# lingfeiwang/normalisr

Hardware: AMD Instinct MI355X
Metric: association tests/sec (gene x gene coex) (higher is better)
Workload: dtype i8 digits x i8 -> i32 exact, 46-bit fixed point, f64 combine (f64 residuals, sums of sq...

## Files before the change

### include/normalisr_hip.h

```cpp
#ifndef NORMALISR_HIP_H
#define NORMALISR_HIP_H

#include <stdint.h>

#ifdef __cplusplus
extern "C" {
#endif

#define NRM_F32 0
#define NRM_F64 1

#define NRM_OK 0
#define NRM_E_ARG -1
#define NRM_E_DEVICE -2
#define NRM_E_NUMERIC -3
#define NRM_E_UNSUPPORTED -4

#define NRM_ROW_TILE 128
#define NRM_K_TILE 16

#define NRM_PCOEF 20

int nrm_version(void);
const char* nrm_last_error(void);
// ... 14 lines not shown
					const double* d_c, int64_t nc, int64_t ldc, const double* d_dci, int rank,
					double* d_out, int64_t ldo, int64_t rows_pad,
					double* d_ss, double* d_coef, void* stream);

#define NRM_FIX_STRIDE 8
int nrm_residualize_q(const void* d_x, int x_dtype, int64_t rows, int64_t n, int64_t ldx,
					  const double* d_c, int64_t nc, int64_t ldc, const double* d_dci, int rank,
					  double* d_out, int64_t ldo, int64_t rows_pad, double* d_ss, double* d_coef,
					  int nslices, void* d_q, int32_t* d_exp, int64_t plane_pitch_bytes, const double* d_cmax, double* d_fix, void* stream);
int nrm_binnet_debug_buffer(void* d_stamps);
int nrm_residualize_q_chunked(const void* d_x, int x_dtype, int64_t rows, int64_t n, int64_t ldx,
							  const double* d_c, int64_t nc, int64_t ldc, const double* d_dci, int rank,
							  int64_t rows_pad, double* d_ss, int nslices, void* d_q, int32_t* d_exp,
							  int64_t chunk_ksteps, const double* d_cmax, double* d_fix, void* stream);

int nrm_gram_f64(const double* d_a, const double* d_b, int64_t m_pad, int64_t n_pad, int64_t k_pad,
				 int64_t lda, int64_t ldb, double* d_dot, int64_t ldd, int symmetric,
				 int64_t m_rows, int64_t n_rows, void* d_work, void* stream);
int nrm_gram_f64_band(const double* d_a, const double* d_b, int64_t m_pad, int64_t n_pad, int64_t k_pad,
					  int64_t lda, int64_t ldb, double* d_dot, int64_t ldd, int symmetric,
					  int64_t m_rows, int64_t n_rows, int64_t row0, int64_t row1, void* d_work, void* stream);
int64_t nrm_gram_workspace_bytes(void);

int64_t nrm_quant_bytes(int64_t rows_pad, int64_t k_pad, int nslices);
int nrm_quantize_rows(const double* d_x, int64_t rows_pad, int64_t k_pad, int64_t ldx, int nslices, void* d_q, int32_t* d_exp,
					  double* d_fix , int64_t n_cells , void* stream);
int nrm_gram_i8_band(const void* d_qa, const int32_t* d_ea, int64_t plane_a_bytes, const void* d_qb, const int32_t* d_eb,
					 int64_t plane_b_bytes, int64_t m_pad, int64_t n_pad, int64_t k_pad, int nslices, double* d_dot, int64_t ldd,
					 int symmetric, int64_t m_rows, int64_t n_rows, int64_t row0, int64_t row1, void* d_work, void* stream);
int nrm_gram_i8_chunk(const void* d_qa, const int32_t* d_ea, int64_t plane_a_bytes, const void* d_qb, const int32_t* d_eb,
					  int64_t plane_b_bytes, int64_t m_pad, int64_t n_pad, int64_t k_pad, int nslices, double* d_dot, int64_t ldd,
					  int symmetric, int64_t m_rows, int64_t n_rows, int accumulate, int64_t b_block_rows, int64_t b_block_stride_bytes,
					  int b_first, int b_count, void* d_work, void* stream);

typedef struct nrm_pvalue_plan {
	double a;
	double alpha;
	double ln_front;
	double umax;
	double coef[NRM_PCOEF];
} nrm_pvalue_plan;
int nrm_pvalue_plan_init(nrm_pvalue_plan* plan, double dof);
int nrm_pvalue_plan_init_many(const double* dof, int64_t count, double* out, int64_t pitch);
int nrm_pvalue_plan_fill_many(const double* dof, int64_t count, double* out, int64_t pitch);

int nrm_pvalues_from_r2(const double* d_r2, int64_t count, double dof, double* d_p, void* stream);

int nrm_assoc_sweep(const double* d_dot, int64_t ldd, const double* d_ssx, const double* d_ssy,
					int64_t nx, int64_t ny, int64_t n_cells, double dof, int symmetric, int stat_kind,
					void* d_p, void* d_stat, void* d_r, void* d_t, int out_dtype, int64_t ldo,
					int32_t* d_flags, int fix_nslices, const double* d_fixx, const double* d_fixy, double guard_tol, void* stream);
int nrm_assoc_sweep_band(const double* d_dot, int64_t ldd, const double* d_ssx, const double* d_ssy,
						 int64_t nx, int64_t ny, int64_t n_cells, double dof, int symmetric, int stat_kind,
						 void* d_p, void* d_stat, void* d_r, void* d_t, int out_dtype, int64_t ldo,
						 int32_t* d_flags, int64_t row0, int64_t row1, int fix_nslices, const double* d_fixx, const double* d_fixy,
						 double guard_tol, void* stream);

int nrm_assoc_sweep_mirror(const double* d_dot, int64_t ldd, const double* d_ssx, const double* d_ssy, int64_t mx, int64_t my,
						   int64_t n_cells, double dof, void* d_p, void* d_stat, int out_dtype, int64_t ldo, int64_t r0, int64_t c0,
						   int32_t* d_flags, int fix_nslices, const double* d_fixx, const double* d_fixy, double guard_tol, void* stream);

int nrm_alpha(const void* d_stat, int stat_dtype, int64_t ldg, int stat_kind, const double* d_ssx, int64_t n_cells,
			  const double* d_bx, const double* d_by, int64_t nx, int64_t ny, int64_t nc, void* d_alpha, int out_dtype,
			  void* stream);

int64_t nrm_design_products_workspace_doubles(int64_t rows, int64_t n_cells);
// ... 297 lines not shown
```

### normalisr_amd/_lib.py

```python
import ctypes
import os
import sys

HERE = os.path.dirname(os.path.abspath(__file__))
LIB_PATH = os.path.join(HERE, 'libnormalisr_hip.so')

NRM_F32, NRM_F64 = 0, 1
NRM_TSV_I64, NRM_TSV_I32, NRM_TSV_U8 = 16, 17, 18
NRM_I64, NRM_I32, NRM_U8, NRM_I16 = 16, 17, 18, 19
NRM_S1_COMMON, NRM_S1_SKIP = -2, -1
DESIGN_NOTONE, DESIGN_NEG, DESIGN_GT1, DESIGN_HAS1, DESIGN_NAN = 1, 2, 4, 8, 16
DESIGN_CSR_BAD = 5
NRM_E_ARG, NRM_E_DEVICE, NRM_E_NUMERIC, NRM_E_UNSUPPORTED = -1, -2, -3, -4
ROW_TILE, K_TILE, PCOEF, FIX_STRIDE = 128, 16, 20, 8

_i64, _i32, _vp, _dbl = ctypes.c_int64, ctypes.c_int, ctypes.c_void_p, ctypes.c_double


class PvaluePlan(ctypes.Structure):
	_fields_ = [('a', _dbl), ('alpha', _dbl), ('ln_front', _dbl), ('umax', _dbl), ('coef', _dbl * PCOEF)]


_SIGNATURES = {
	'nrm_version': ([], _i32),
	'nrm_last_error': ([], ctypes.c_char_p),
	'nrm_device_count': ([ctypes.POINTER(_i32)], _i32),
	'nrm_set_device': ([_i32], _i32),
	'nrm_release_cache': ([], _i32),
	'nrm_last_guard': ([ctypes.POINTER(_i64), ctypes.POINTER(_dbl)], _i32),
	'nrm_host_pin': ([_vp, _i64, _i32], _i32),
	'nrm_host_unpin': ([_vp], _i32),
	'nrm_copy_to_host': ([_vp, _vp, _i64, _vp], _i32),
	'nrm_host_alloc': ([ctypes.POINTER(_vp), _i64], _i32),
	'nrm_host_free': ([_vp], _i32),
	'nrm_fill_zero': ([_vp, _i64, _vp], _i32),
	'nrm_fill_i32': ([_vp, _i32, _i64, _vp], _i32),
	'nrm_copy_rows': ([_vp, _i64, _vp, _i64, _i64, _i64, _vp], _i32),
	'nrm_residualize': ([_vp, _i32, _i64, _i64, _i64, _vp, _i64, _i64, _vp, _i32, _vp, _i64, _i64, _vp, _vp, _vp], _i32),
	'nrm_residualize_q': ([_vp, _i32, _i64, _i64, _i64, _vp, _i64, _i64, _vp, _i32, _vp, _i64, _i64, _vp, _vp, _i32, _vp, _vp, _i64, _vp, _vp, _vp], _i32),
	'nrm_binnet_debug_buffer': ([_vp], _i32),
	'nrm_residualize_q_chunked': ([_vp, _i32, _i64, _i64, _i64, _vp, _i64, _i64, _vp, _i32, _i64, _vp, _i32, _vp, _vp, _i64, _vp, _vp, _vp], _i32),
	'nrm_gram_f64': ([_vp, _vp, _i64, _i64, _i64, _i64, _i64, _vp, _i64, _i32, _i64, _i64, _vp, _vp], _i32),
	'nrm_gram_f64_band': ([_vp, _vp, _i64, _i64, _i64, _i64, _i64, _vp, _i64, _i32, _i64, _i64, _i64, _i64, _vp, _vp], _i32),
	'nrm_gram_workspace_bytes': ([], _i64),
	'nrm_quant_bytes': ([_i64, _i64, _i32], _i64),
	'nrm_quantize_rows': ([_vp, _i64, _i64, _i64, _i32, _vp, _vp, _vp, _i64, _vp], _i32),
	'nrm_gram_i8_band': ([_vp, _vp, _i64, _vp, _vp, _i64, _i64, _i64, _i64, _i32, _vp, _i64, _i32, _i64, _i64, _i64, _i64, _vp, _vp], _i32),
	'nrm_gram_i8_chunk': ([_vp, _vp, _i64, _vp, _vp, _i64, _i64, _i64, _i64, _i32, _vp, _i64, _i32, _i64, _i64, _i32, _i64, _i64, _i32, _i32, _vp, _vp], _i32),
	'nrm_pvalue_plan_init': ([ctypes.POINTER(PvaluePlan), _dbl], _i32),
	'nrm_pvalue_plan_init_many': ([_vp, _i64, _vp, _i64], _i32),
	'nrm_pvalue_plan_fill_many': ([_vp, _i64, _vp, _i64], _i32),
	'nrm_pvalues_from_r2': ([_vp, _i64, _dbl, _vp, _vp], _i32),
	'nrm_assoc_sweep': ([_vp, _i64, _vp, _vp, _i64, _i64, _i64, _dbl, _i32, _i32, _vp, _vp, _vp, _vp, _i32, _i64, _vp, _i32, _vp, _vp, _dbl, _vp], _i32),
	'nrm_assoc_sweep_band': ([_vp, _i64, _vp, _vp, _i64, _i64, _i64, _dbl, _i32, _i32, _vp, _vp, _vp, _vp, _i32, _i64, _vp, _i64, _i64, _i32, _vp, _vp, _dbl, _vp], _i32),
	'nrm_assoc_sweep_mirror': ([_vp, _i64, _vp, _vp, _i64, _i64, _i64, _dbl, _vp, _vp, _i32, _i64, _i64, _i64, _vp, _i32, _vp, _vp, _dbl, _vp], _i32),
	'nrm_host_mirror_rows': ([_vp, _i64, _i32, _i64, _i64, _i32], _i32),
	'nrm_copy_rect_to_host': ([_vp, _i64, _vp, _i64, _i64, _i64, _vp], _i32),
	'nrm_single4_sweep': ([_vp, _vp, _i64, _vp, _vp, _i64, _i64, _i64, _i64, _dbl, _i32, _vp, _vp, _vp, _i32, _i64, _vp, _vp, _vp], _i32),
	'nrm_gram_i8_fix_dot': ([_vp, _i64, _vp, _vp, _i64, _i64, _i32, _i64, _vp], _i32),
	'nrm_single4_sweep_guarded': ([_vp, _vp, _i64, _vp, _vp, _i64, _i64, _i64, _i64, _dbl, _i32, _vp, _vp, _vp, _i32, _i64, _vp, _vp,
								  _vp, _vp, _dbl, _dbl, _i32, _dbl, _vp, _vp], _i32),
	'nrm_spd_prepare': ([_vp, _i64, _i64, _i64, _vp, _vp, _vp, _vp], _i32),
	'nrm_spd_start': ([_vp, _i64, _i32, _vp, _vp, _vp], _i32),
	'nrm_spd_transpose_residual': ([_vp, _i64, _vp, _vp, _vp, _vp], _i32),
	'nrm_spd_update': ([_vp, _vp, _i64, _vp], _i32),
	'nrm_spd_finish': ([_vp, _i64, _i64, _vp, _vp, _vp, _vp], _i32),
	'nrm_single4_design_scalars': ([_vp, _i64, _i64, _vp, _vp, _vp, _vp], _i32),
	'nrm_design_products_workspace_doubles': ([_i64, _i64], _i64),
	'nrm_design_products': ([_vp, _i32, _i64, _i64, _i64, _vp, _i64, _i64, _vp, _vp, _i32, _vp], _i32),
	'nrm_residualize_wide': ([_vp, _i32, _i64, _i64, _i64, _vp, _i64, _i64, _vp, _vp, _i32, _vp, _i64, _vp, _vp, _vp, _i32, _vp], _i32),
	'nrm_gram_skinny': ([_vp, _i32, _i64, _i64, _i64, _vp, _i64, _i64, _vp, _vp, _i64, _i64, _dbl, _vp, _vp], _i32),
	'nrm_gram_skinny_workspace_bytes': ([], _i64),
	'nrm_de_small_sweep': ([_vp, _vp, _vp, _i64, _i32, _vp, _i64, _i64, _i64, _dbl, _i32, _vp, _vp, _vp, _vp, _i32, _i64, _vp, _vp, _vp, _i32, _vp], _i32),
	'nrm_single1_sweep': ([_vp, _i64, _vp, _i64, _vp, _i64, _i64, _i64, _i64, _i32, _vp, _vp, _vp, _vp, _i32, _i64, _vp, _vp], _i32),
	'nrm_de_sparse_chunk': ([], _i64),
	'nrm_de_sparse_max_covariates': ([], _i64),
	'nrm_de_sparse_fused_covariates': ([], _i64),
	'nrm_de_sparse_ct_doubles': ([_i64, _i64, _i64], _i64),
	'nrm_de_sparse': ([_vp, _i32, _i64, _i64, _i64, _vp, _i64, _vp, _vp, _vp, _vp, _vp, _vp, _i64, _vp, _vp, _i64, _vp, _i64, _i32, _vp, _vp, _vp, _vp, _i64, _i64, _dbl, _vp, _vp], _i32),
	'nrm_design_count': ([_vp, _i32, _i64, _i64, _i64, _vp, _i64, _vp, _vp], _i32),
	'nrm_design_plan': ([_vp, _i64, _i64, _i64, _vp, _vp, _vp, _vp, _vp, _vp, _vp, _vp, _vp], _i32),
# ... 207 lines not shown
```

### normalisr_amd/csrc/nrm_gram_i8.hip

```cpp
#include <type_traits>
#include "nrm_gram_sched.h"
#include "nrm_digits.h"
#include "nrm_fix.h"

#define QK 32
#define QCHUNK 512
#define QD 3
#ifndef QI_EDGE
#define QI_EDGE 0
#endif
#ifndef QI_EXP
#define QI_EXP 0
#endif

typedef int i4_t __attribute__((ext_vector_type(4)));
typedef int i16_t __attribute__((ext_vector_type(16)));

template <bool HAZARD>
__device__ __forceinline__ void q_dma16_s(const char* sbase, unsigned lane16, unsigned lds_dst) {
	if (HAZARD)
		asm volatile("s_nop 4\n\ts_mov_b32 m0, %2\n\ts_nop 0\n\tglobal_load_lds_dwordx4 %1, %0" ::"s"(sbase), "v"(lane16), "s"(lds_dst) : "m0");
	else
		asm volatile("s_mov_b32 m0, %2\n\ts_nop 0\n\tglobal_load_lds_dwordx4 %1, %0" ::"s"(sbase), "v"(lane16), "s"(lds_dst) : "m0");
}

template <int NS>
__global__ void __launch_bounds__(256) k_quantize_rows(const double* __restrict__ X, int64_t kx, int64_t ldx, char* __restrict__ Q,
													   int64_t plane_bytes, int64_t nks, int* __restrict__ exps, double* __restrict__ fix, double n_cells) {
	constexpr int B = 8 * NS - 2;
	const int lane = threadIdx.x & 63;
	const int64_t row = (int64_t)blockIdx.x * 4 + (threadIdx.x >> 6);
	const double* x = X + row * ldx;
	double mx = 0.0, ssq = 0.0;
	for (int64_t k = (int64_t)lane * 2; k < kx; k += 128) {
		const d2_t v = *reinterpret_cast<const d2_t*>(x + k);
		mx = fmax(mx, fmax(fabs(v[0]), fabs(v[1])));
		ssq = fma(v[0], v[0], fma(v[1], v[1], ssq));
	}
#pragma unroll
	for (int o = 32; o > 0; o >>= 1) mx = fmax(mx, __shfl_xor(mx, o, 64));
	int e = 0;
	if (mx > 0.0 && mx < INFINITY) (void)frexp(mx, &e);
	const int sh = e - B;
	if (lane == 0) exps[row] = sh;
	const int64_t ib = row >> 5;
	const int r = (int)(row & 31);
	char* qrow = Q + (ib * nks) * 1024 + (2 * r) * 16;
	const int flip = (r >> 3) & 1;
	int dsum[NS - 1];
	unsigned dsq[NS - 1];
	unsigned long long dsq64[NS - 1];
	unsigned steps = 0;
#pragma unroll
	for (int s = 0; s < NS - 1; s++) {
		dsum[s] = 0;
		dsq[s] = 0u;
// ... 20 lines not shown
			dsum[s] = __builtin_amdgcn_sdot4((int)w[s], 0x01010101, dsum[s], false);
			dsq[s] = (unsigned)__builtin_amdgcn_sdot4((int)w[s], (int)w[s], (int)dsq[s], false);
		}
		if ((++steps & 0x7fff) == 0) {
#pragma unroll
			for (int s = 0; s < NS - 1; s++) {
				dsq64[s] += dsq[s];
				dsq[s] = 0u;
			}
		}
	}
	if (fix) {
		double S[5] = {0, 0, 0, 0, 0}, Q2[5] = {0, 0, 0, 0, 0};
#pragma unroll
		for (int s = 0; s < NS - 1; s++) {
			S[s] = (double)wave_sum_i32(dsum[s]);
			unsigned long long q = dsq64[s] + dsq[s];
#pragma unroll
			for (int o = 32; o > 0; o >>= 1) q += __shfl_xor(q, o, 64);
			Q2[s] = (double)q;
		}
#pragma unroll
		for (int o = 32; o > 0; o >>= 1) ssq += __shfl_xor(ssq, o, 64);
		if (lane == 0) nrm_fix_record<NS>(fix + row * NRM_FIX_STRIDE, S, Q2, sh, ssq, n_cells);
	}
}

struct BBlocks {
	int rows;
	int first, count;
	int64_t stride;
};

template <int NS>
__device__ __forceinline__ void gram_piece_i8(const char* __restrict__ QA, const char* __restrict__ QB, int64_t plane_a, int64_t plane_b,
											  int64_t nks, const int* __restrict__ ea, const int* __restrict__ eb, double* __restrict__ C,
											  int64_t ldc, int ti, int tj, int k0, int k1, double* __restrict__ slab, int m_rows, int n_rows,
											  int symmetric, int accumulate, int edge_tj, BBlocks bb, const char* lds, unsigned lds0) {
	constexpr int STAGE = 8 * NS * 1024;
	const int tid = threadIdx.x, lane = tid & 63;
	const int wid = __builtin_amdgcn_readfirstlane(tid >> 6);
	const int wm = wid >> 2, wn = wid & 3;
	const char* qb_t = QB + ((int64_t)tj * 4 * nks) * 1024;
	const int* eb_t = eb + tj * GN;
	if (bb.rows) {
		const int blk = tj * GN / bb.rows, within = tj * GN - blk * bb.rows, wb = (bb.first + blk) % bb.count;
		qb_t = QB + wb * bb.stride + ((int64_t)(within / 32) * nks) * 1024;
		eb_t = eb + wb * bb.rows + within;
	}
	const bool host = symmetric && ti == tj && ti < edge_tj;
	const bool hw = host && wm == 1 && wn < 2;
	const char* src_w = wid < 4 ? QA + (((int64_t)ti * 4 + wid) * nks) * 1024
								: (host && wid == 4) ? QB + ((int64_t)edge_tj * 4 * nks) * 1024 : qb_t + ((int64_t)(wid - 4) * nks) * 1024;
	const unsigned src_hi = (unsigned)__builtin_amdgcn_readfirstlane((int)((uint64_t)src_w >> 32)),
				   src_lo = (unsigned)__builtin_amdgcn_readfirstlane((int)(uint64_t)src_w);
	const char* src0 = reinterpret_cast<const char*>((uint64_t)src_hi << 32 | (uint64_t)src_lo);
	const unsigned lane16 = lane * 16;
	const int64_t plane = wid < 4 ? plane_a : plane_b;
	const unsigned dst0 = lds0 + wid * NS * 1024;
	auto issue_one = [&](int buf, int ks, int s, auto hazard) {
		if (QI_EXP & 1) return;
		if (QI_EXP & 2) ks &= 3;
		q_dma16_s<decltype(hazard)::value>(src0 + s * plane + (int64_t)ks * 1024, lane16, dst0 + buf * STAGE + s * 1024);
	};
	auto issue = [&](int buf, int ks) {
#pragma unroll
		for (int s = 0; s < NS; s++) issue_one(buf, ks, s, std::true_type{});
	};
	i16_t acc[NS][2];
	auto clear = [&]() {
#pragma unroll
		for (int w = 0; w < NS; w++)
#pragma unroll
			for (int i = 0; i < 2; i++)
#pragma unroll
				for (int j = 0; j < 16; j++) acc[w][i][j] = 0;
	};
	const int r = lane & 31;
	const int pos = (2 * r + ((lane >> 5) ^ ((r >> 3) & 1))) * 16;
	const bool diag = symmetric && ti == tj;
	const bool edge = QI_EDGE && !diag && tj * GN + 32 >= n_rows;
	const int a_blk = edge ? (wid & 3) : hw ? wn * 2 : wm * 2, b_blk = edge ? 0 : wn;
	const int b_slot = hw ? 4 : (host && wid == 0) ? 0 : 4 + b_blk;
	const int aoff = a_blk * NS * 1024 + pos;
	const int boff = b_slot * NS * 1024 + pos;
	const int row_w = ti * GM + a_blk * 32, col_w = hw ? edge_tj * GN : tj * GN + b_blk * 32;
	bool want[2];
#pragma unroll
	for (int i = 0; i < 2; i++) want[i] = row_w + i * 32 < m_rows && col_w < n_rows && (!diag || col_w + 31 >= row_w + i * 32);
	if (edge) {
		want[0] = want[0] && wid < 4;
		want[1] = false;
	}
	double* cbase;
	int64_t pitch;
	if (slab) {
		cbase = slab + ((hw ? wm * 2 : a_blk) * 32) * GN + b_blk * 32;
		pitch = GN;
	} else {
		cbase = C + (int64_t)row_w * ldc + col_w;
		pitch = ldc;
	}
	cbase += (int64_t)(4 * (lane >> 5)) * pitch + (lane & 31);
	const int* ea_l = ea + row_w + 4 * (lane >> 5);
	const int eb_l = hw ? eb[edge_tj * GN + (lane & 31)] : eb_t[b_blk * 32 + (lane & 31)];
	auto flush = [&](bool first) {
#pragma unroll
		for (int i = 0; i < 2; i++) {
			if (!want[i]) continue;
#pragma unroll
			for (int q = 0; q < 16; q++) {
				const int rr = i * 32 + (q & 3) + 8 * (q >> 2);
				long long lo = 0, hi = 0;
#pragma unroll
				for (int w = 0; w < NS; w++) {
					if (w < 3)
						lo += (long long)acc[w][i][q] << (8 * w);
					else
						hi += (long long)acc[w][i][q] << (8 * (w - 3));
				}
				double v = fma((double)hi, 16777216.0, (double)lo);
				v = ldexp(v, ea_l[rr] + eb_l + 8 * (NS - 1));
				double* o = cbase + (int64_t)rr * pitch;
				*o = (first && !(accumulate && !slab)) ? v : *o + v;
			}
		}
	};
	clear();
	__syncthreads();
	if (k0 >= k1) return;
	issue(0, k0);
	issue(1, min(k0 + 1, k1 - 1));
	int in_chunk = 0;
	bool first = true;
	auto kloop = [&](auto mask) {
	constexpr int MASK = decltype(mask)::value;
	for (int ks = k0; ks < k1; ks++) {
		const int buf = (ks - k0) % QD;
		asm volatile("s_waitcnt vmcnt(%0)" ::"i"(NS) : "memory");
		if (!(QI_EXP & 4)) __syncthreads();
		const char* st = lds + buf * STAGE;
		const int nbuf = (ks - k0 + 2) % QD, nks = min(ks + 2, k1 - 1);
		i4_t fa[NS][2], fb[NS];
		auto read_row = [&](int s) {
#pragma unroll
			for (int i = 0; i < 2; i++)
				if (MASK >> i & 1) fa[s][i] = *reinterpret_cast<const i4_t*>(st + aoff + (i * NS + s) * 1024);
			fb[NS - 1 - s] = *reinterpret_cast<const i4_t*>(st + boff + (NS - 1 - s) * 1024);
		};
		auto mfma_row = [&](int s, int t0, int t1) {
#pragma unroll
			for (int t = t0; t < t1; t++)
#pragma unroll
				for (int i = 0; i < 2; i++)
					if (MASK >> i & 1)
						acc[s + t - (NS - 1)][i] = __builtin_amdgcn_mfma_i32_32x32x32_i8(fa[s][i], fb[t], acc[s + t - (NS - 1)][i], 0, 0, 0);
		};
		auto dma = [&](int j) {
			__builtin_amdgcn_sched_barrier(0);
			issue_one(nbuf, nks, j, std::false_type{});
			__builtin_amdgcn_sched_barrier(0);
		};
		if (MASK) {
			read_row(0);
			read_row(1);
#pragma unroll
			for (int s = 0; s < NS - 1; s++) {
				mfma_row(s, NS - 1 - s, NS);
				dma(s);
				if (s + 2 < NS) read_row(s + 2);
			}
			mfma_row(NS - 1, 0, NS / 2);
			dma(NS - 1);
			mfma_row(NS - 1, NS / 2, NS);
		} else {
#pragma unroll
			for (int s = 0; s < NS; s++) dma(s);
		}
		if (MASK && ++in_chunk == QCHUNK && ks + 1 < k1) {
			flush(first);
			first = false;
			clear();
			in_chunk = 0;
		}
	}
	};
	if (QI_EDGE && want[0] && !want[1])
		kloop(std::integral_constant<int, 1>{});
	else if (want[0] || want[1])
		kloop(std::integral_constant<int, 3>{});
	else
		kloop(std::integral_constant<int, 0>{});
	asm volatile("s_waitcnt vmcnt(0)" ::: "memory");
	flush(first);
}

template <int NS>
__global__ void __launch_bounds__(512) k_gram_i8(const char* __restrict__ QA, const char* __restrict__ QB, int64_t plane_a, int64_t plane_b,
												 int64_t nks, const int* __restrict__ ea, const int* __restrict__ eb, double* __restrict__ C,
												 int64_t ldc, int symmetric, GramSched s, BBlocks bb) {
	__shared__ __attribute__((aligned(1024))) char lds[QD * 8 * NS * 1024];
	typedef __attribute__((address_space(3))) char* lds_ptr_t;
	const unsigned lds0 = __builtin_amdgcn_readfirstlane((unsigned)(size_t)(lds_ptr_t)lds);
	gram_for_each_piece(s, [&](int t, int k0, int k1, double* slab) {
		int ti, tj;
		gram_sched_coords(s, t, symmetric, ti, tj);
		gram_piece_i8<NS>(QA, QB, plane_a, plane_b, nks, ea, eb, C, ldc, ti, tj, k0, k1, slab, s.m_rows, s.n_rows, symmetric, s.accumulate, s.fold,
						  bb, lds, lds0);
	});
}

static int g_num_cu_q = 0;

extern "C" int64_t nrm_quant_bytes(int64_t rows_pad, int64_t k_pad, int nslices) {
	if (rows_pad < 0 || k_pad < 0 || nslices < 1) return 0;
	const int64_t nks = (k_pad + QK - 1) / QK;
	return (rows_pad / 32) * nks * 1024 * nslices;
}

extern "C" int nrm_quantize_rows(const double* d_x, int64_t rows_pad, int64_t k_pad, int64_t ldx, int nslices, void* d_q, int32_t* d_exp,
								 double* d_fix, int64_t n_cells, void* stream) {
	NRM_REQUIRE(nslices == 5 || nslices == 6, "nrm_quantize_rows: 5 or 6 slices");
	NRM_REQUIRE(rows_pad >= 0 && rows_pad % 32 == 0 && k_pad > 0 && k_pad % 16 == 0 && ldx >= k_pad && ldx % 2 == 0,
				"nrm_quantize_rows: rows must be padded to 32 (%d for nrm_gram_i8), cells to 16", GM);
	if (rows_pad == 0) return NRM_OK;
	NRM_REQUIRE(d_x && d_q && d_exp && (uintptr_t)d_x % 16 == 0 && (uintptr_t)d_q % 16 == 0, "nrm_quantize_rows: null or misaligned pointer");
	NRM_REQUIRE(!d_fix || (n_cells > 0 && n_cells <= k_pad && k_pad < (1 << 22)), "nrm_quantize_rows: row records need 0 < n_cells <= k_pad < 2^22");
	const int64_t nks = (k_pad + QK - 1) / QK;
	const int64_t plane = (rows_pad / 32) * nks * 1024;
	dim3 grid((unsigned)(rows_pad / 4));
	if (nslices == 5)
		hipLaunchKernelGGL(k_quantize_rows<5>, grid, dim3(256), 0, (hipStream_t)stream, d_x, k_pad, ldx, (char*)d_q, plane, nks, d_exp, d_fix, (double)n_cells);
	else
		hipLaunchKernelGGL(k_quantize_rows<6>, grid, dim3(256), 0, (hipStream_t)stream, d_x, k_pad, ldx, (char*)d_q, plane, nks, d_exp, d_fix, (double)n_cells);
	return nrm_check_launch("k_quantize_rows");
}

static int gram_i8_impl(const void* d_qa, const int32_t* d_ea, int64_t plane_a_bytes, const void* d_qb, const int32_t* d_eb,
						int64_t plane_b_bytes, int64_t m_pad, int64_t n_pad, int64_t k_pad, int nslices, double* d_dot, int64_t ldd,
						int symmetric, int64_t m_rows, int64_t n_rows, int64_t row0, int64_t row1, int accumulate, BBlocks bb, bool may_fold, void* d_work, void* stream) {
	NRM_REQUIRE(nslices == 5 || nslices == 6, "nrm_gram_i8: 5 or 6 slices");
	NRM_REQUIRE(m_pad >= 0 && n_pad >= 0 && k_pad > 0 && m_pad % GM == 0 && n_pad % GN == 0, "nrm_gram_i8: sizes must be padded to %d", GM);
	NRM_REQUIRE(ldd >= n_pad && ldd % 2 == 0, "nrm_gram_i8: pitch too small");
	NRM_REQUIRE(!symmetric || m_pad == n_pad, "nrm_gram_i8: symmetric needs square output");
	NRM_REQUIRE(row0 >= 0 && row0 <= row1 && row1 <= m_pad && row0 % (GSB * GM) == 0 && (row1 % (GSB * GM) == 0 || row1 == m_pad),
				"nrm_gram_i8_band: rows [row0, row1) must be cut at multiples of %d", GSB * GM);
	if (m_pad == 0 || n_pad == 0 || row0 == row1) return NRM_OK;
	NRM_REQUIRE(d_qa && d_qb && d_ea && d_eb && d_dot && d_work, "nrm_gram_i8: null pointer");
	if (g_num_cu_q == 0) {
		int dev = 0;
		NRM_HIP(hipGetDevice(&dev));
		NRM_HIP(hipDeviceGetAttribute(&g_num_cu_q, hipDeviceAttributeMultiprocessorCount, dev));
		if (g_num_cu_q <= 0) g_num_cu_q = 256;
	}
	const int64_t nks = (k_pad + QK - 1) / QK;
	const int64_t plane_a = plane_a_bytes ? plane_a_bytes : (m_pad / 32) * nks * 1024,
				  plane_b = plane_b_bytes ? plane_b_bytes : ((bb.rows ? bb.rows : n_pad) / 32) * nks * 1024;
	NRM_REQUIRE(plane_a >= (m_pad / 32) * nks * 1024 && plane_b >= ((bb.rows ? bb.rows : n_pad) / 32) * nks * 1024,
				"nrm_gram_i8: plane pitch smaller than the operand");
	GramSched s;
	if (may_fold && symmetric && !accumulate && bb.rows == 0 && d_qa == d_qb && d_ea == d_eb && plane_a == plane_b && !nrm_debug_is("gram_fold", "0"))
		NRM_TRY(gram_plan_fold(s, m_pad, n_pad, nks, symmetric, m_rows, n_rows, row0, row1, g_num_cu_q, (double*)d_work));
	else
		NRM_TRY(gram_plan(s, m_pad, n_pad, nks, symmetric, m_rows, n_rows, row0, row1, g_num_cu_q, (double*)d_work));
	s.accumulate = accumulate ? 1 : 0;
	if (nslices == 5)
		hipLaunchKernelGGL(k_gram_i8<5>, dim3((unsigned)s.nwg), dim3(512), 0, (hipStream_t)stream, (const char*)d_qa, (const char*)d_qb, plane_a,
						   plane_b, nks, d_ea, d_eb, d_dot, ldd, symmetric, s, bb);
	else
		hipLaunchKernelGGL(k_gram_i8<6>, dim3((unsigned)s.nwg), dim3(512), 0, (hipStream_t)stream, (const char*)d_qa, (const char*)d_qb, plane_a,
						   plane_b, nks, d_ea, d_eb, d_dot, ldd, symmetric, s, bb);
	if (s.tiles_al + s.tiles_sk > 0)
		hipLaunchKernelGGL(k_gram_fixup<1>, dim3((unsigned)(s.tiles_al + s.tiles_sk), GM / GFIX_ROWS), dim3(256), 0, (hipStream_t)stream, d_dot, ldd, symmetric, s);
	return nrm_check_launch("k_gram_i8");
}

extern "C" int nrm_gram_i8_band(const void* d_qa, const int32_t* d_ea, int64_t plane_a_bytes, const void* d_qb, const int32_t* d_eb,
								int64_t plane_b_bytes, int64_t m_pad, int64_t n_pad, int64_t k_pad, int nslices, double* d_dot, int64_t ldd,
								int symmetric, int64_t m_rows, int64_t n_rows, int64_t row0, int64_t row1, void* d_work, void* stream) {
	return gram_i8_impl(d_qa, d_ea, plane_a_bytes, d_qb, d_eb, plane_b_bytes, m_pad, n_pad, k_pad, nslices, d_dot, ldd, symmetric, m_rows, n_rows, row0,
						row1, 0, BBlocks{0, 0, 1, 0}, true, d_work, stream);
}

extern "C" int nrm_gram_i8_chunk(const void* d_qa, const int32_t* d_ea, int64_t plane_a_bytes, const void* d_qb, const int32_t* d_eb,
								 int64_t plane_b_bytes, int64_t m_pad, int64_t n_pad, int64_t k_pad, int nslices, double* d_dot, int64_t ldd,
								 int symmetric, int64_t m_rows, int64_t n_rows, int accumulate, int64_t b_block_rows, int64_t b_block_stride_bytes,
								 int b_first, int b_count, void* d_work, void* stream) {
	BBlocks bb{0, 0, 1, 0};
	if (b_block_rows) {
		NRM_REQUIRE(!symmetric && b_block_rows > 0 && b_block_rows % GN == 0 && n_pad % b_block_rows == 0 && b_count > 0 && b_first >= 0 &&
						b_first < b_count && n_pad / b_block_rows <= b_count && b_block_stride_bytes % 16 == 0 && b_block_rows < (1 << 30),
					"nrm_gram_i8_chunk: bad block description of operand B");
		bb = BBlocks{(int)b_block_rows, b_first, b_count, b_block_stride_bytes};
	}
	return gram_i8_impl(d_qa, d_ea, plane_a_bytes, d_qb, d_eb, plane_b_bytes, m_pad, n_pad, k_pad, nslices, d_dot, ldd, symmetric, m_rows, n_rows, 0,
						m_pad, accumulate, bb, false, d_work, stream);
}
```

### normalisr_amd/csrc/nrm_host_logic.h

```cpp
#pragma once
#include <algorithm>
#include <cmath>
#include <cstdint>
#include <cstring>
#include <mutex>
#include <vector>
#include "../../include/normalisr_hip.h"

#if defined(__HIPCC__)
#define NRM_HD __host__ __device__
#else
#define NRM_HD
#endif

void nrm_set_error(const char* fmt, ...);
#ifndef NRM_REQUIRE
#define NRM_REQUIRE(cond, ...)      \
	do {                            \
		if (!(cond)) {              \
			nrm_set_error(__VA_ARGS__); \
			return NRM_E_ARG;       \
		}                           \
	} while (0)
#endif
// ... 41 lines not shown
					li = 0;
					int len = h;
					while (t >= len) {
						t -= len;
						li++;
						len--;
					}
					lj = li + t;
				}
				ti = bi * GSB + li;
				tj = bj * GSB + lj;
				return;
			}
			t -= cnt;
		}
	}
	ti = 0;
	tj = 0;
}

struct GramSched {
	int m_rows, n_rows;
	int ntm, ntn;
	int nkt;
	int tiles_dp;
	int tiles_al;
	int parts;
	int tiles_sk;
	int units_per_wg;
	int nwg;
	int tile0;
	int accumulate;
	int fold;
	double* work;
};

NRM_HD inline __attribute__((always_inline)) void gram_sched_coords(const GramSched& s, int t, int symmetric, int& ti, int& tj) {
	if (!s.fold) {
		gram_tile_coords(s.tile0 + t, symmetric, s.ntm, s.ntn, ti, tj);
		return;
	}
	const int lead = s.fold;
	if (t < lead * (lead + 1) / 2)
		gram_tile_coords(t, 1, lead, lead, ti, tj);
	else
		ti = tj = lead;
}
NRM_HD inline bool gram_is_host(const GramSched& s, int ti, int tj) { return ti == tj && ti < s.fold; }

template <typename F>
NRM_HD inline __attribute__((always_inline)) void gram_pieces_of(const GramSched& s, int block, F piece) {
	const int per_xcd = s.nwg >> 3;
	const int p = (block & 7) * per_xcd + (block >> 3);
	int t_dp = p;
	bool al_todo = p < s.tiles_al * s.parts;
	int64_t u = (int64_t)p * s.units_per_wg;
	const int64_t total = (int64_t)s.tiles_sk * s.nkt;
	int64_t uend = u + s.units_per_wg;
	if (uend > total) uend = total;
	int sk_piece = 0;
	for (;;) {
		int t, k0, k1;
		double* slab = nullptr;
		if (t_dp < s.tiles_dp) {
			t = t_dp;
			k0 = 0;
			k1 = s.nkt;
			t_dp += s.nwg;
		} else if (al_todo) {
			al_todo = false;
			const int ta = p / s.parts, part = p - ta * s.parts;
			t = s.tiles_dp + ta;
			k0 = (int)((int64_t)s.nkt * part / s.parts);
			k1 = (int)((int64_t)s.nkt * (part + 1) / s.parts);
			slab = s.work + (int64_t)p * (GM * GN);
		} else if (u < uend) {
			const int ts = (int)(u / s.nkt);
			k0 = (int)(u - (int64_t)ts * s.nkt);
			int64_t k1l = k0 + (uend - u);
			k1 = k1l > s.nkt ? s.nkt : (int)k1l;
			t = s.tiles_dp + s.tiles_al + ts;
			u += k1 - k0;
			if (!(k0 == 0 && k1 == s.nkt)) slab = s.work + ((int64_t)s.tiles_al * s.parts + 2 * p + sk_piece) * (GM * GN);
			sk_piece++;
		} else {
			break;
		}
		piece(t, k0, k1, slab);
	}
}

static inline int64_t nrm_host_gram_workspace_doubles(int nwg) { return (int64_t)3 * nwg * GM * GN; }

static inline int64_t gram_tiles_before(int64_t bi, int symmetric, int64_t ntm, int64_t ntn) {
	const int64_t nbn = (ntn + GSB - 1) / GSB;
	int64_t t = 0;
	for (int64_t b = 0; b < bi; b++) {
		const int64_t h = std::min<int64_t>(GSB, ntm - b * GSB);
		for (int64_t bj = symmetric ? b : 0; bj < nbn; bj++) {
			const int64_t w = std::min<int64_t>(GSB, ntn - bj * GSB);
			t += (symmetric && b == bj) ? h * (h + 1) / 2 : h * w;
		}
	}
	return t;
}

static inline void gram_split_phases(GramSched& s, int64_t tiles) {
	const int64_t waves = tiles / s.nwg, rem = tiles - waves * s.nwg;
	s.tiles_dp = (int)(waves * s.nwg);
	s.parts = 1;
	s.tiles_al = 0;
	for (int parts = 2; parts <= 8 && s.nkt >= 8 * parts; parts *= 2)
		if (rem >= s.nwg / parts) {
			s.parts = parts;
			s.tiles_al = s.nwg / parts;
			break;
		}
	const int64_t sk = rem - s.tiles_al;
	s.tiles_sk = (int)sk;
	s.units_per_wg = (int)((sk * s.nkt + s.nwg - 1) / s.nwg);
}

static inline int gram_plan(GramSched& s, int64_t m_pad, int64_t n_pad, int64_t nkt, int symmetric, int64_t m_rows, int64_t n_rows, int64_t row0,
							int64_t row1, int nwg, double* work) {
	const int64_t ntm = m_pad / GM, ntn = n_pad / GN;
	NRM_REQUIRE((symmetric ? ntn * (ntn + 1) / 2 : ntm * ntn) < (1LL << 30), "nrm_gram: problem too large for one launch");
	const int64_t tile0 = gram_tiles_before(row0 / (GSB * GM), symmetric, ntm, ntn);
	const int64_t tiles = gram_tiles_before((row1 + GSB * GM - 1) / (GSB * GM), symmetric, ntm, ntn) - tile0;
	NRM_REQUIRE(tiles < (1LL << 30) && nkt < (1LL << 30), "nrm_gram: problem too large for one launch");
	s.tile0 = (int)tile0;
	s.accumulate = 0;
	s.fold = 0;
	s.m_rows = (int)((m_rows > 0 && m_rows < m_pad) ? m_rows : m_pad);
	s.n_rows = (int)((n_rows > 0 && n_rows < n_pad) ? n_rows : n_pad);
	s.ntm = (int)ntm;
	s.ntn = (int)ntn;
	s.nkt = (int)nkt;
	s.nwg = nwg - nwg % 8;
	gram_split_phases(s, tiles);
	s.work = work;
	return NRM_OK;
}

static inline int gram_plan_fold(GramSched& s, int64_t m_pad, int64_t n_pad, int64_t nkt, int symmetric, int64_t m_rows, int64_t n_rows, int64_t row0,
								 int64_t row1, int nwg, double* work) {
	const int rc = gram_plan(s, m_pad, n_pad, nkt, symmetric, m_rows, n_rows, row0, row1, nwg, work);
	if (rc != NRM_OK) return rc;
	const int valid = s.n_rows - (s.ntn - 1) * GN;
	if (symmetric && row0 == 0 && row1 == m_pad && s.ntn >= 2 && s.ntm == s.ntn && s.m_rows == s.n_rows && valid >= 1 && valid <= 32) {
		s.fold = s.ntn - 1;
		gram_split_phases(s, (int64_t)(s.ntn - 1) * s.ntn / 2 + 1);
	}
	return NRM_OK;
}

static const double kNrmH[] = {1.0,
							-0.02083333333333333333333,
							0.000390625,
							-0.000007879670965608465608466,
							1.696766579172178130511e-7,
							-3.805064191721906565657e-9,
							8.748377596315407304061e-11,
							-2.044523359411973817584e-12,
							4.833351797967704408319e-14,
							-1.152434101767385923873e-15,
// ... 118 lines not shown
```

Baseline: 5.630 billion.

## Chain DMA prefetch across consecutive gram pieces and restructure flush

Replaces the per-piece callback loop with a cursor that looks ahead to the next piece. While the current piece's last k-steps run, it issues the next piece's first loads into the rotating LDS buffers, so the per-piece barrier and pipeline refill are skipped. The flush now combines the i8 digit planes with f64 FMAs and batches the loads of old output values. Row exponents are staged through a small added LDS region. Timestamp instrumentation compiled under QI_PHASES is also added. Chaining adds phase bookkeeping and a small LDS increase, and it can be switched off with a debug flag.

```diff
diff --git a/include/normalisr_hip.h b/include/normalisr_hip.h
--- a/include/normalisr_hip.h
+++ b/include/normalisr_hip.h
@@ -70,6 +70,7 @@
 					  int64_t plane_b_bytes, int64_t m_pad, int64_t n_pad, int64_t k_pad, int nslices, double* d_dot, int64_t ldd,
 					  int symmetric, int64_t m_rows, int64_t n_rows, int accumulate, int64_t b_block_rows, int64_t b_block_stride_bytes,
 					  int b_first, int b_count, void* d_work, void* stream);
+int nrm_k2_debug_buffer(void* d_stamps);
 
 typedef struct nrm_pvalue_plan {
 	double a;
diff --git a/normalisr_amd/_lib.py b/normalisr_amd/_lib.py
--- a/normalisr_amd/_lib.py
+++ b/normalisr_amd/_lib.py
@@ -47,6 +47,7 @@
 	'nrm_quantize_rows': ([_vp, _i64, _i64, _i64, _i32, _vp, _vp, _vp, _i64, _vp], _i32),
 	'nrm_gram_i8_band': ([_vp, _vp, _i64, _vp, _vp, _i64, _i64, _i64, _i64, _i32, _vp, _i64, _i32, _i64, _i64, _i64, _i64, _vp, _vp], _i32),
 	'nrm_gram_i8_chunk': ([_vp, _vp, _i64, _vp, _vp, _i64, _i64, _i64, _i64, _i32, _vp, _i64, _i32, _i64, _i64, _i32, _i64, _i64, _i32, _i32, _vp, _vp], _i32),
+	'nrm_k2_debug_buffer': ([_vp], _i32),
 	'nrm_pvalue_plan_init': ([ctypes.POINTER(PvaluePlan), _dbl], _i32),
 	'nrm_pvalue_plan_init_many': ([_vp, _i64, _vp, _i64], _i32),
 	'nrm_pvalue_plan_fill_many': ([_vp, _i64, _vp, _i64], _i32),
diff --git a/normalisr_amd/csrc/nrm_gram_i8.hip b/normalisr_amd/csrc/nrm_gram_i8.hip
--- a/normalisr_amd/csrc/nrm_gram_i8.hip
+++ b/normalisr_amd/csrc/nrm_gram_i8.hip
@@ -12,6 +12,10 @@
 #ifndef QI_EXP
 #define QI_EXP 0
 #endif
+#ifndef QI_PHASES
+#define QI_PHASES 0
+#endif
+#define QP_MAX 16
 
 typedef int i4_t __attribute__((ext_vector_type(4)));
 typedef int i16_t __attribute__((ext_vector_type(16)));
@@ -22,6 +26,18 @@
 		asm volatile("s_nop 4\n\ts_mov_b32 m0, %2\n\ts_nop 0\n\tglobal_load_lds_dwordx4 %1, %0" ::"s"(sbase), "v"(lane16), "s"(lds_dst) : "m0");
 	else
 		asm volatile("s_mov_b32 m0, %2\n\ts_nop 0\n\tglobal_load_lds_dwordx4 %1, %0" ::"s"(sbase), "v"(lane16), "s"(lds_dst) : "m0");
+}
+
+__device__ __forceinline__ long long q_stamp() {
+#if QI_PHASES
+	long long t;
+	__builtin_amdgcn_sched_barrier(0);
+	asm volatile("s_memrealtime %0\n\ts_waitcnt lgkmcnt(0)" : "=s"(t)::"memory");
+	__builtin_amdgcn_sched_barrier(0);
+	return t;
+#else
+	return 0;
+#endif
 }
 
 template <int NS>
@@ -108,40 +124,57 @@
 	int64_t stride;
 };
 
-template <int NS>
-__device__ __forceinline__ void gram_piece_i8(const char* __restrict__ QA, const char* __restrict__ QB, int64_t plane_a, int64_t plane_b,
-											  int64_t nks, const int* __restrict__ ea, const int* __restrict__ eb, double* __restrict__ C,
-											  int64_t ldc, int ti, int tj, int k0, int k1, double* __restrict__ slab, int m_rows, int n_rows,
-											  int symmetric, int accumulate, int edge_tj, BBlocks bb, const char* lds, unsigned lds0) {
-	constexpr int STAGE = 8 * NS * 1024;
-	const int tid = threadIdx.x, lane = tid & 63;
-	const int wid = __builtin_amdgcn_readfirstlane(tid >> 6);
-	const int wm = wid >> 2, wn = wid & 3;
+__device__ __forceinline__ const char* gram_wave_src(const char* __restrict__ QA, const char* __restrict__ QB, int64_t nks, int ti, int tj, int symmetric,
+													 int edge_tj, const BBlocks& bb, int wid) {
 	const char* qb_t = QB + ((int64_t)tj * 4 * nks) * 1024;
-	const int* eb_t = eb + tj * GN;
 	if (bb.rows) {
 		const int blk = tj * GN / bb.rows, within = tj * GN - blk * bb.rows, wb = (bb.first + blk) % bb.count;
 		qb_t = QB + wb * bb.stride + ((int64_t)(within / 32) * nks) * 1024;
-		eb_t = eb + wb * bb.rows + within;
 	}
 	const bool host = symmetric && ti == tj && ti < edge_tj;
-	const bool hw = host && wm == 1 && wn < 2;
 	const char* src_w = wid < 4 ? QA + (((int64_t)ti * 4 + wid) * nks) * 1024
 								: (host && wid == 4) ? QB + ((int64_t)edge_tj * 4 * nks) * 1024 : qb_t + ((int64_t)(wid - 4) * nks) * 1024;
 	const unsigned src_hi = (unsigned)__builtin_amdgcn_readfirstlane((int)((uint64_t)src_w >> 32)),
 				   src_lo = (unsigned)__builtin_amdgcn_readfirstlane((int)(uint64_t)src_w);
-	const char* src0 = reinterpret_cast<const char*>((uint64_t)src_hi << 32 | (uint64_t)src_lo);
+	return reinterpret_cast<const char*>((uint64_t)src_hi << 32 | (uint64_t)src_lo);
+}
+
+struct PieceLink {
+	const char* src;
+	const char* tail;
+	int tail_mask;
+	int phase;
+	bool chained_in;
+};
+
+template <int NS>
+__device__ __forceinline__ void gram_piece_i8(const int* __restrict__ ea, const int* __restrict__ eb, int64_t plane_a, int64_t plane_b, double* __restrict__ C,
+											  int64_t ldc, int ti, int tj, int k0, int k1, double* __restrict__ slab, int m_rows, int n_rows,
+											  int symmetric, int accumulate, int edge_tj, BBlocks bb, PieceLink link, char* lds, unsigned lds0, long long* stamps, int piece_idx) {
+	constexpr int STAGE = 8 * NS * 1024;
+	const long long t_entry = q_stamp();
+	long long t_first = 0;
+	const int tid = threadIdx.x, lane = tid & 63;
+	const int wid = __builtin_amdgcn_readfirstlane(tid >> 6);
+	const int wm = wid >> 2, wn = wid & 3;
+	const int* eb_t = eb + tj * GN;
+	if (bb.rows) {
+		const int blk = tj * GN / bb.rows, within = tj * GN - blk * bb.rows, wb = (bb.first + blk) % bb.count;
+		eb_t = eb + wb * bb.rows + within;
+	}
+	const bool host = symmetric && ti == tj && ti < edge_tj;
+	const bool hw = host && wm == 1 && wn < 2;
+	const char* src0 = link.src;
 	const unsigned lane16 = lane * 16;
 	const int64_t plane = wid < 4 ? plane_a : plane_b;
 	const unsigned dst0 = lds0 + wid * NS * 1024;
-	auto issue_one = [&](int buf, int ks, int s, auto hazard) {
+	auto issue_one = [&](int buf, const char* src, int s, auto hazard) {
 		if (QI_EXP & 1) return;
-		if (QI_EXP & 2) ks &= 3;
-		q_dma16_s<decltype(hazard)::value>(src0 + s * plane + (int64_t)ks * 1024, lane16, dst0 + buf * STAGE + s * 1024);
+		q_dma16_s<decltype(hazard)::value>(src + s * plane, lane16, dst0 + buf * STAGE + s * 1024);
 	};
 	auto issue = [&](int buf, int ks) {
 #pragma unroll
-		for (int s = 0; s < NS; s++) issue_one(buf, ks, s, std::true_type{});
+		for (int s = 0; s < NS; s++) issue_one(buf, src0 + (int64_t)((QI_EXP & 2) ? ks & 3 : ks) * 1024, s, std::true_type{});
 	};
 	i16_t acc[NS][2];
 	auto clear = [&]() {
@@ -178,45 +211,67 @@
 		pitch = ldc;
 	}
 	cbase += (int64_t)(4 * (lane >> 5)) * pitch + (lane & 31);
-	const int* ea_l = ea + row_w + 4 * (lane >> 5);
+	const int ea_w = ea[row_w + ((QI_EDGE && edge) ? (lane & 31) : lane)];
 	const int eb_l = hw ? eb[edge_tj * GN + (lane & 31)] : eb_t[b_blk * 32 + (lane & 31)];
+	int* const ex_w = reinterpret_cast<int*>(lds + QD * STAGE) + wid * 64;
 	auto flush = [&](bool first) {
-#pragma unroll
-		for (int i = 0; i < 2; i++) {
-			if (!want[i]) continue;
-#pragma unroll
-			for (int q = 0; q < 16; q++) {
-				const int rr = i * 32 + (q & 3) + 8 * (q >> 2);
-				long long lo = 0, hi = 0;
-#pragma unroll
-				for (int w = 0; w < NS; w++) {
-					if (w < 3)
-						lo += (long long)acc[w][i][q] << (8 * w);
-					else
-						hi += (long long)acc[w][i][q] << (8 * (w - 3));
-				}
-				double v = fma((double)hi, 16777216.0, (double)lo);
-				v = ldexp(v, ea_l[rr] + eb_l + 8 * (NS - 1));
-				double* o = cbase + (int64_t)rr * pitch;
-				*o = (first && !(accumulate && !slab)) ? v : *o + v;
+		ex_w[lane] = ea_w;
+		const int* ex_l = ex_w + 4 * (lane >> 5);
+		auto value = [&](int i, int q) {
+			double lo = (double)acc[2][i][q], hi = (double)acc[NS - 1][i][q];
+			lo = fma(lo, 256.0, (double)acc[1][i][q]);
+			lo = fma(lo, 256.0, (double)acc[0][i][q]);
+#pragma unroll
+			for (int w = NS - 2; w >= 3; w--) hi = fma(hi, 256.0, (double)acc[w][i][q]);
+			const int rr = i * 32 + (q & 3) + 8 * (q >> 2);
+			return ldexp(fma(hi, 16777216.0, lo), ex_l[rr] + eb_l + 8 * (NS - 1));
+		};
+		if (first && !(accumulate && !slab)) {
+#pragma unroll
+			for (int i = 0; i < 2; i++) {
+				if (!want[i]) continue;
+#pragma unroll
+				for (int q = 0; q < 16; q++) cbase[(int64_t)(i * 32 + (q & 3) + 8 * (q >> 2)) * pitch] = value(i, q);
+			}
+		} else {
+#pragma unroll
+			for (int i = 0; i < 2; i++) {
+				if (!want[i]) continue;
+				double old[16];
+#pragma unroll
+				for (int q = 0; q < 16; q++) old[q] = cbase[(int64_t)(i * 32 + (q & 3) + 8 * (q >> 2)) * pitch];
+#pragma unroll
+				for (int q = 0; q < 16; q++) cbase[(int64_t)(i * 32 + (q & 3) + 8 * (q >> 2)) * pitch] = old[q] + value(i, q);
 			}
 		}
 	};
 	clear();
-	__syncthreads();
-	if (k0 >= k1) return;
-	issue(0, k0);
-	issue(1, min(k0 + 1, k1 - 1));
+	if (!link.chained_in) {
+		__syncthreads();
+		issue(0, k0);
+		issue(1, min(k0 + 1, k1 - 1));
+	}
 	int in_chunk = 0;
 	bool first = true;
+	if (QI_PHASES) {
+		asm volatile("s_waitcnt vmcnt(%0)" ::"i"(NS) : "memory");
+		__builtin_amdgcn_s_barrier();
+		t_first = q_stamp();
+	}
 	auto kloop = [&](auto mask) {
 	constexpr int MASK = decltype(mask)::value;
-	for (int ks = k0; ks < k1; ks++) {
-		const int buf = (ks - k0) % QD;
+	int ks = k0;
+#pragma nounroll
+	for (int pass = 0; pass < 2; pass++) {
+	const int kend = pass ? k1 : max(k0, k1 - 2);
+	const char* nsrc = pass ? link.tail + (int64_t)((ks + 2 - k1) & link.tail_mask) * 1024 : src0 + (int64_t)(k0 + 2) * 1024;
+	const int nstep = pass ? (1024 & link.tail_mask) : 1024;
+	for (; ks < kend; ks++, nsrc += nstep) {
+		const int buf = (ks - k0 + link.phase) % QD;
 		asm volatile("s_waitcnt vmcnt(%0)" ::"i"(NS) : "memory");
 		if (!(QI_EXP & 4)) __syncthreads();
 		const char* st = lds + buf * STAGE;
-		const int nbuf = (ks - k0 + 2) % QD, nks = min(ks + 2, k1 - 1);
+		const int nbuf = (ks - k0 + 2 + link.phase) % QD;
 		i4_t fa[NS][2], fb[NS];
 		auto read_row = [&](int s) {
 #pragma unroll
@@ -234,7 +289,7 @@
 		};
 		auto dma = [&](int j) {
 			__builtin_amdgcn_sched_barrier(0);
-			issue_one(nbuf, nks, j, std::false_type{});
+			issue_one(nbuf, (QI_EXP & 2) ? src0 + (int64_t)((ks + 2) & 3) * 1024 : nsrc, j, std::false_type{});
 			__builtin_amdgcn_sched_barrier(0);
 		};
 		if (MASK) {
@@ -260,6 +315,7 @@
 			in_chunk = 0;
 		}
 	}
+	}
 	};
 	if (QI_EDGE && want[0] && !want[1])
 		kloop(std::integral_constant<int, 1>{});
@@ -267,26 +323,81 @@
 		kloop(std::integral_constant<int, 3>{});
 	else
 		kloop(std::integral_constant<int, 0>{});
+	const long long t_exit = q_stamp();
 	asm volatile("s_waitcnt vmcnt(0)" ::: "memory");
+	const long long t_drain = q_stamp();
 	flush(first);
+	if (QI_PHASES && stamps && piece_idx < QP_MAX - 1) {
+		asm volatile("s_waitcnt vmcnt(0)" ::: "memory");
+		const long long t_flush = q_stamp();
+		if (tid == 0) {
+			long long* o = stamps + ((int64_t)blockIdx.x * QP_MAX + piece_idx) * 8;
+			o[0] = t_entry;
+			o[1] = t_first;
+			o[2] = t_exit;
+			o[3] = t_drain;
+			o[4] = t_flush;
+			o[5] = k0;
+			o[6] = k1;
+			o[7] = (long long)(ti * 65536 + tj) * 4 + (slab ? 1 : 0) + (host ? 2 : 0);
+		}
+	}
 }
 
 template <int NS>
 __global__ void __launch_bounds__(512) k_gram_i8(const char* __restrict__ QA, const char* __restrict__ QB, int64_t plane_a, int64_t plane_b,
 												 int64_t nks, const int* __restrict__ ea, const int* __restrict__ eb, double* __restrict__ C,
-												 int64_t ldc, int symmetric, GramSched s, BBlocks bb) {
-	__shared__ __attribute__((aligned(1024))) char lds[QD * 8 * NS * 1024];
+												 int64_t ldc, int symmetric, GramSched s, BBlocks bb, long long* stamps) {
+	__shared__ __attribute__((aligned(1024))) char lds[QD * 8 * NS * 1024 + 8 * 256];
 	typedef __attribute__((address_space(3))) char* lds_ptr_t;
 	const unsigned lds0 = __builtin_amdgcn_readfirstlane((unsigned)(size_t)(lds_ptr_t)lds);
-	gram_for_each_piece(s, [&](int t, int k0, int k1, double* slab) {
-		int ti, tj;
-		gram_sched_coords(s, t, symmetric, ti, tj);
-		gram_piece_i8<NS>(QA, QB, plane_a, plane_b, nks, ea, eb, C, ldc, ti, tj, k0, k1, slab, s.m_rows, s.n_rows, symmetric, s.accumulate, s.fold,
-						  bb, lds, lds0);
-	});
+	const int wid = __builtin_amdgcn_readfirstlane(threadIdx.x >> 6);
+	GramPieceCursor cur(s, (int)blockIdx.x);
+	GramPiece g, gn;
+	bool have = cur.next(s, g);
+	int ti = 0, tj = 0, piece_idx = 0;
+	PieceLink link{nullptr, nullptr, 0, 0, false};
+	if (have) {
+		gram_sched_coords(s, g.t, symmetric, ti, tj);
+		link.src = gram_wave_src(QA, QB, nks, ti, tj, symmetric, s.fold, bb, wid);
+	}
+	while (have) {
+		const bool have_n = cur.next(s, gn);
+		int tin = 0, tjn = 0;
+		const char* src_n = link.src;
+		if (have_n) {
+			gram_sched_coords(s, gn.t, symmetric, tin, tjn);
+			src_n = gram_wave_src(QA, QB, nks, tin, tjn, symmetric, s.fold, bb, wid);
+		}
+		const bool chain = s.chain && have_n && g.k1 - g.k0 >= 2 && gn.k1 - gn.k0 >= 2;
+		link.tail = chain ? src_n + (int64_t)gn.k0 * 1024 : link.src + (int64_t)(g.k1 - 1) * 1024;
+		link.tail_mask = chain ? -1 : 0;
+		gram_piece_i8<NS>(ea, eb, plane_a, plane_b, C, ldc, ti, tj, g.k0, g.k1, g.slab, s.m_rows, s.n_rows, symmetric, s.accumulate, s.fold, bb, link, lds, lds0,
+						  stamps, piece_idx);
+		piece_idx++;
+		link.phase = chain ? (link.phase + g.k1 - g.k0) % QD : 0;
+		link.chained_in = chain;
+		link.src = src_n;
+		g = gn;
+		ti = tin;
+		tj = tjn;
+		have = have_n;
+	}
+	if (QI_PHASES && stamps && threadIdx.x == 0) {
+		long long* o = stamps + ((int64_t)blockIdx.x * QP_MAX + min(piece_idx, QP_MAX - 1)) * 8;
+		o[0] = q_stamp();
+		o[6] = -1;
+	}
 }
 
 static int g_num_cu_q = 0;
+static long long* g_k2_stamps = nullptr;
+
+extern "C" int nrm_k2_debug_buffer(void* d_stamps) {
+	NRM_REQUIRE(QI_PHASES || !d_stamps, "nrm_k2_debug_buffer: this library was built without -DQI_PHASES=1");
+	g_k2_stamps = (long long*)d_stamps;
+	return NRM_OK;
+}
 
 extern "C" int64_t nrm_quant_bytes(int64_t rows_pad, int64_t k_pad, int nslices) {
 	if (rows_pad < 0 || k_pad < 0 || nslices < 1) return 0;
@@ -340,12 +451,13 @@
 	else
 		NRM_TRY(gram_plan(s, m_pad, n_pad, nks, symmetric, m_rows, n_rows, row0, row1, g_num_cu_q, (double*)d_work));
 	s.accumulate = accumulate ? 1 : 0;
+	s.chain = nrm_debug_is("gram_chain", "0") ? 0 : 1;
 	if (nslices == 5)
 		hipLaunchKernelGGL(k_gram_i8<5>, dim3((unsigned)s.nwg), dim3(512), 0, (hipStream_t)stream, (const char*)d_qa, (const char*)d_qb, plane_a,
-						   plane_b, nks, d_ea, d_eb, d_dot, ldd, symmetric, s, bb);
+						   plane_b, nks, d_ea, d_eb, d_dot, ldd, symmetric, s, bb, g_k2_stamps);
 	else
 		hipLaunchKernelGGL(k_gram_i8<6>, dim3((unsigned)s.nwg), dim3(512), 0, (hipStream_t)stream, (const char*)d_qa, (const char*)d_qb, plane_a,
-						   plane_b, nks, d_ea, d_eb, d_dot, ldd, symmetric, s, bb);
+						   plane_b, nks, d_ea, d_eb, d_dot, ldd, symmetric, s, bb, g_k2_stamps);
 	if (s.tiles_al + s.tiles_sk > 0)
 		hipLaunchKernelGGL(k_gram_fixup<1>, dim3((unsigned)(s.tiles_al + s.tiles_sk), GM / GFIX_ROWS), dim3(256), 0, (hipStream_t)stream, d_dot, ldd, symmetric, s);
 	return nrm_check_launch("k_gram_i8");
diff --git a/normalisr_amd/csrc/nrm_host_logic.h b/normalisr_amd/csrc/nrm_host_logic.h
--- a/normalisr_amd/csrc/nrm_host_logic.h
+++ b/normalisr_amd/csrc/nrm_host_logic.h
@@ -97,6 +97,7 @@
 	int tile0;
 	int accumulate;
 	int fold;
+	int chain;
 	double* work;
 };
 
@@ -155,6 +156,55 @@
 	}
 }
 
+struct GramPiece {
+	int t, k0, k1;
+	double* slab;
+};
+struct GramPieceCursor {
+	int p, t_dp, sk_piece;
+	bool al_todo;
+	int64_t u, uend;
+	NRM_HD inline __attribute__((always_inline)) GramPieceCursor(const GramSched& s, int block) {
+		const int per_xcd = s.nwg >> 3;
+		p = (block & 7) * per_xcd + (block >> 3);
+		t_dp = p;
+		al_todo = p < s.tiles_al * s.parts;
+		u = (int64_t)p * s.units_per_wg;
+		const int64_t total = (int64_t)s.tiles_sk * s.nkt;
+		uend = u + s.units_per_wg;
+		if (uend > total) uend = total;
+		sk_piece = 0;
+	}
+	NRM_HD inline __attribute__((always_inline)) bool next(const GramSched& s, GramPiece& g) {
+		if (t_dp < s.tiles_dp) {
+			g.t = t_dp;
+			g.k0 = 0;
+			g.k1 = s.nkt;
+			g.slab = nullptr;
+			t_dp += s.nwg;
+		} else if (al_todo) {
+			al_todo = false;
+			const int ta = p / s.parts, part = p - ta * s.parts;
+			g.t = s.tiles_dp + ta;
+			g.k0 = (int)((int64_t)s.nkt * part / s.parts);
+			g.k1 = (int)((int64_t)s.nkt * (part + 1) / s.parts);
+			g.slab = s.work + (int64_t)p * (GM * GN);
+		} else if (u < uend) {
+			const int ts = (int)(u / s.nkt);
+			g.k0 = (int)(u - (int64_t)ts * s.nkt);
+			const int64_t k1l = g.k0 + (uend - u);
+			g.k1 = k1l > s.nkt ? s.nkt : (int)k1l;
+			g.t = s.tiles_dp + s.tiles_al + ts;
+			u += g.k1 - g.k0;
+			g.slab = (g.k0 == 0 && g.k1 == s.nkt) ? nullptr : s.work + ((int64_t)s.tiles_al * s.parts + 2 * p + sk_piece) * (GM * GN);
+			sk_piece++;
+		} else {
+			return false;
+		}
+		return true;
+	}
+};
+
 static inline int64_t nrm_host_gram_workspace_doubles(int nwg) { return (int64_t)3 * nwg * GM * GN; }
 
 static inline int64_t gram_tiles_before(int64_t bi, int symmetric, int64_t ntm, int64_t ntn) {
@@ -196,6 +246,7 @@
 	s.tile0 = (int)tile0;
 	s.accumulate = 0;
 	s.fold = 0;
+	s.chain = 0;
 	s.m_rows = (int)((m_rows > 0 && m_rows < m_pad) ? m_rows : m_pad);
 	s.n_rows = (int)((n_rows > 0 && n_rows < n_pad) ? n_rows : n_pad);
 	s.ntm = (int)ntm;
```

New measurement: 5.655 billion (median of 5 runs). No clear change (+0.4%).
